# sirpkt/flink-tensorflow

Hardware: AMD Instinct MI355X
Metric: records/sec (whole node) + p50 per-record latency, ResNet-50 stream DP=1/8 (higher is better)
Workload: dtype bf16

## Files before the change

flink_tensorflow_amd/config.py:

```python
from __future__ import annotations

import argparse
import contextlib
import dataclasses
import os
from dataclasses import dataclass, field
from typing import Any

_HBM_BYTES_MI355X = 288 * 1024 ** 3


@dataclass
class EngineConfig:
    parallelism: int = 1
    max_batch: int = 256
    max_delay_ms: float = 10.0
    precision: str = "bf16"
    batch_buckets: tuple = (64, 256)
    arena_fraction: float = 0.9
    use_hip_graph: bool = True
    pipeline_depth: int = 3
    checkpoint_interval_s: float | None = None
    checkpoint_dir: str | None = None
    restart_attempts: int = 0
    restart_delay_s: float = 0.0
    channel_capacity: int = 1024
    log_level: str = "INFO"
    sibling_conv_fusion: bool = True
    fuse_preprocess_stem: bool = True
    fuse_block_tails: bool = True
    decimate_tails: bool = True
    recompute_tails: bool = True
    chain_max_links: int = 2
    pw_res_kernel: bool = True
    conv3x3c64_kernel: bool = True
    chain_batch: int = -1
    chain_min_hw: int = 5041
    chain_edge: bool = True
    wd_fused_step: bool = True
    wd_sparse_exchange: str = "owner"
    wd_bucket_slack: float = 2.0
    extra: dict = field(default_factory=dict)

    @classmethod
    def field_names(cls) -> list[str]:
        return [f.name for f in dataclasses.fields(cls) if f.name != "extra"]

    def _coerce(self, name: str, value: Any) -> Any:
        cur = getattr(self, name)
        typ = {f.name: f.type for f in dataclasses.fields(self)}[name]
        if value is None:
            return None
        if isinstance(value, str):
            if "tuple" in str(typ):
                return tuple(int(v) for v in value.replace(" ", "").split(",") if v)
            if "bool" in str(typ):
                return value.lower() in ("1", "true", "yes", "on")
            if "int" in str(typ) and "float" not in str(typ):
                return int(value)
            if "float" in str(typ):
                return float(value)
            return value
        if isinstance(cur, tuple) and isinstance(value, (list, tuple)):
            return tuple(value)
        return value

    def update(self, values: dict) -> "EngineConfig":
        for k, v in values.items():
            if k in self.field_names():
                setattr(self, k, self._coerce(k, v))
            else:
                self.extra[k] = v
        self.validate()
        return self

    @classmethod
    def from_yaml(cls, path: str, base: "EngineConfig | None" = None) -> "EngineConfig":
        import yaml

        with open(path) as f:
            data = yaml.safe_load(f) or {}
        return (base or cls()).update(data)

    @classmethod
    def from_env(cls, base: "EngineConfig | None" = None, prefix: str = "FT_", environ=None) -> "EngineConfig":
        environ = os.environ if environ is None else environ
        vals = {}
# ... 101 lines not shown
```

flink_tensorflow_amd/graph/compiler.py:

```python
from __future__ import annotations

import collections
import logging
import types
from typing import Any

import numpy as np
import torch

from ..ops import fp8 as F8
from ..ops import kernels as K
from ..types.dtypes import DataType
from ..types.names import TensorName
from ..types.tensor import StringTensor
from ..utils import tracing
from . import ops_core
from .conv_lowering import _ACTS, ConvLowering
from .graph import Graph, Node
from .op_registry import OpContext, lookup
from .ops_nn import same_pads
from .plan import CompileError, Step, Val, _buf_shape, _cfg, _coff, _eff_scale, _host, _nbytes, _root, _target, _view
from .transformer_lowering import TransformerLowering

__all__ = ["CompiledFunction", "CompileError", "Step", "Val", "compile_signature"]

LOG = logging.getLogger("flink_tensorflow_amd.compiler")

_STATS = ("fused_shortcuts", "fused_tails", "decimated_tails", "fused_pools", "conv3x3c64", "pw_res", "chained_tails",
          "conv_lite", "commuted_pools", "sibling_groups", "fused_preprocess")

_BINARY = {"Add": "add", "AddV2": "add", "Sub": "sub", "Mul": "mul", "RealDiv": "div", "Div": "div",
           "Maximum": "max", "Minimum": "min"}


class _ConstSession:

    def __init__(self, variables):
        self.variables = variables
        self._const_cache = {}


class CompiledFunction(TransformerLowering, ConvLowering):
    def __init__(self, graph: Graph, feeds: dict[str, tuple[tuple, Any]], fetches: list[str], device,
                 variables: dict | None = None, use_graph: bool = True, strict: bool = False,
                 topk_fetch: bool = True, precision: str = "bf16", calibration: dict | None = None,
                 arena=None, token_capacity: int | None = None):
        if precision not in ("bf16", "fp8"):
            raise ValueError(f"precision must be bf16 or fp8, not {precision!r}")
        from .control_flow import fold_static_control_flow
        from .functions import has_functional_ops, lower_functional_ops

        if has_functional_ops(graph):
            graph = lower_functional_ops(graph)
        graph = fold_static_control_flow(graph, list(feeds), list(fetches))
        self.graph = graph
        self.arena = arena
        self.token_cap = token_capacity
        self._pack: dict | None = None
        self._cls_nodes: set[str] = set()
        self._cur_cls = False
        self._cls_cache: dict[int, Val] = {}
        self.activation_bytes = 0
        self.precision = precision
        self.device = torch.device(device)
        if self.device.type != "cuda":
            use_graph = False
        self.feed_names = [str(TensorName.parse(f)) for f in feeds]
        self.feed_specs = {str(TensorName.parse(f)): v for f, v in feeds.items()}
        self.fetch_names = [str(TensorName.parse(f)) for f in fetches]
        self.variables = variables or {}
        self.strict = strict
        self.steps: list[Step] = []
        self.params: list[torch.Tensor] = []
        self.glue_ops: list[str] = []
        self.vals: dict[tuple[str, int], Val] = {}
        self._fused: set[str] = set()
        self._const_sess = _ConstSession(self.variables)
        self._input_bufs: dict[str, torch.Tensor] = {}
        self._outputs: list = []
        self._graph_obj: torch.cuda.CUDAGraph | None = None
        self._graph_tail: torch.cuda.CUDAGraph | None = None
        self._head: tuple[str, Step] | None = None
# ... 720 lines not shown
                    born[id(tgt)] = i
        for t in owners.values():
            t.last_use = max([t.last_use] + [c.last_use for c in getattr(t, "_concat_children", [])])
        transient = []
        for k, t in owners.items():
            if k in internal:
                continue
            if k in keep:
                t.buf = self._persistent(_buf_shape(t), t.dtype)
            else:
                transient.append(t)
        sizes = [_nbytes(_buf_shape(t), t.dtype) for t in transient]
        first = [born[id(t)] for t in transient]
        last = [max(born[id(t)], t.last_use) for t in transient]
        if chain:
            i0, i1 = chain["range"]
            for j, t in enumerate(transient):
                if id(t) in chain["touched"]:
                    if i0 <= first[j] < i1:
                        first[j] = i0
                    if last[j] >= i0:
                        last[j] = max(last[j], i1 - 1)
            chain_layout = self._plan_chain(chain, born)
            sizes.append(max(chain_layout[1], 1))
            first.append(i0)
            last.append(i1 - 1)
        offs, total = plan_offsets(sizes, first, last)
        self.activation_bytes = total
        slab = self.arena.shared_slab(total) if self.arena is not None else \
            torch.empty(max(total, 1), dtype=torch.uint8, device=self.device)
        for t, off, nb, lu in zip(transient, offs, sizes, last):
            t.buf = slab[off:off + nb].view(t.dtype).view(tuple(_buf_shape(t)))
            self._poison_after.setdefault(lu, []).append(t.buf)
        if chain:
            self._bind_chain(chain, chain_layout, slab, offs[-1])
        for v in self.vals.values():
            if v.alias_of is not None:
                r = _root(v)
                if r.buf is not None:
                    shape = v.shape if id(r) not in internal else (chain["batch"], *v.shape[1:])
                    v.buf = r.buf.view(shape) if r.buf.is_contiguous() else r.buf.reshape(shape)
        if chain:
            self._chain = (chain["range"][0], chain["range"][1], chain["parts"], chain["batch"],
                           [v for v in chain["vals"] if id(_root(v)) not in internal], chain["n"],
                           [v for v in chain["vals"] if id(_root(v)) in internal and v.buf is not None])
        self._outputs = []
        for fv in fetch_vals:
            if fv.is_const:
                self._outputs.append(fv.const)
            else:
                self._outputs.append(fv)

    _CHAIN_KINDS = ("conv", "gemm", "pool", "elementwise", "conv_fp8", "pool_fp8")
    _PERSISTENT_IMPLS = ("conv3x3c64", "bottleneck_tail", "bottleneck_chain", "pw_res")

    def _find_chain(self, keep: set) -> dict | None:
        cfg = _cfg()
        bs = int(getattr(cfg, "chain_batch", 0) or 0)
        auto = bs < 0
        if auto:
            bs = 32
        if bs == 0 or self._pack is not None or not self.steps or not self.feed_names:
            return None
        tn = TensorName.parse(self.feed_names[0])
        N = self.vals[(tn.name, tn.index)].shape[0] if self.vals[(tn.name, tn.index)].shape else 0
        if not N or -(-N // bs) < 2:
            return None
        min_hw = int(getattr(cfg, "chain_min_hw", 3136))

        edge = bool(getattr(cfg, "chain_edge", False))

        def val_ok(v):
            if v is None or v.is_const:
                return True
            r = _root(v)
            if v.rows is not None or v.concat_slot is not None or r.concat_slot is not None or r.is_const:
                return False
            if len(v.shape) != 4 or v.shape[0] != N:
                return False
            return _buf_shape(r)[0] == N

        def step_ok(st):
            vs = [v for v in list(st.inputs) + list(st.outputs) if v is not None and not v.is_const]
            if st.kind not in self._CHAIN_KINDS or not vs or not all(val_ok(v) for v in vs):
                return False
            if auto and st.meta.get("impl") in self._PERSISTENT_IMPLS:
                return False
            big = [v.shape[1] * v.shape[2] >= min_hw for v in vs]
            return any(big) if edge else all(big)

        start = 1 if self.steps[0].kind == "preprocess" else 0
        best, i = None, start
        while i < len(self.steps):
            if not step_ok(self.steps[i]):
                i += 1
                continue
            j = i
            while j < len(self.steps) and step_ok(self.steps[j]):
                j += 1
            if j - i >= 2 and (best is None or j - i > best[1] - best[0]):
                best = (i, j)
            i = j
        if best is None:
            return None
        i0, i1 = best
        vals, touched = [], set()
        for st in self.steps[i0:i1]:
# ... 280 lines not shown
```

flink_tensorflow_amd/graph/conv_lowering.py:

```python
from __future__ import annotations

from dataclasses import dataclass

import numpy as np
import torch

from ..ops import fp8 as F8
from ..ops import kernels as K
from ..types.names import TensorName
from .graph import Node
from .ops_nn import same_pads
from .plan import CompileError, Val, _cfg, _coff, _eff_scale, _root, _target, _view

_ACTS = {"Relu": K.ACT_RELU, "Relu6": K.ACT_RELU6, "Sigmoid": K.ACT_SIGMOID, "Tanh": K.ACT_TANH}

LITE_FP8_CFG = 11
_PP_MIN_K = 512

_PLAIN_ACTS = (K.ACT_NONE, K.ACT_RELU)


@dataclass(frozen=True)
class ConvSite:

# ... 302 lines not shown
                      splits=splits, ws=ws)

        self._emit(c.node.name, "gemm", run_pp, [c.xin], [c.out], {"impl": "gemm_pp"})
        self._finish_conv(c.last, c.absorbed, c.out)

    def _emit_pw_res(self, c: _ConvJob):
        w_nk = c.w_dev.reshape(c.site.cout, c.site.cin)
        bz = self._zero_bias(c)

        def run_pw(xin=c.xin, out=c.out, res_val=c.res_val, w_nk=w_nk, bz=bz):
            K.pw_res(xin.buf, w_nk, bz, res_val.buf, out=_target(out), out_channel_offset=_coff(out))

        self._emit(c.node.name, "conv", run_pw, [c.xin, c.res_val], [c.out], {"impl": "pw_res"})
        self.stats["pw_res"] += 1
        self._finish_conv(c.last, c.absorbed, c.out)

    def _emit_conv_lite(self, c: _ConvJob):
        s = c.site
        cl = K.ConvPP([(tuple(c.xin.shape), s.kernel, s.stride, (s.pads[0], s.pads[2]), s.dil)], s.cout,
                      tuple(c.out.shape[1:3]), self.device)

        def run_l(xin=c.xin, out=c.out, res_val=c.res_val, cl=cl, w2=c.w_dev.reshape(s.cout, -1), b_dev=c.b_dev):
            cl([xin.buf], w2, b_dev, res_val.buf if res_val is not None else None, s.act, out=_target(out),
               out_channel_offset=_coff(out))

        self.stats["conv_lite"] += 1
        self._emit_single_conv(c, run_l)

    def _emit_igemm(self, c: _ConvJob):
        s = c.site

        def run(xin=c.xin, out=c.out, res_val=c.res_val, w_dev=c.w_dev, b_dev=c.b_dev):
            K.conv2d_nhwc(xin.buf, w_dev, b_dev, res_val.buf if res_val is not None else None, s.stride,
                          s.pads, s.dil, s.act, out=_target(out), out_channel_offset=_coff(out),
                          out_scale=_eff_scale(out) if out.qscale is not None else None)

        self._emit_single_conv(c, run)

    def _emit_single_conv(self, c: _ConvJob, run):
        s = c.site
        shortcut_ok = (s.kernel == (1, 1) and s.stride[0] == s.stride[1] and s.pads == (0, 0, 0, 0) and s.dil == (1, 1)
                       and not s.residual and s.act == K.ACT_NONE and not s.out_fp8 and s.unpadded_cin)
        meta = {"shortcut": dict(x=c.xin, w=c.w_ohwi, bias=c.bias, stride=s.stride[0],
                                 params=[c.w_dev, c.b_dev])} if shortcut_ok else None
        self._emit(c.node.name, "conv", run, [c.xin] + ([c.res_val] if c.res_val else []), [c.out], meta)
        self._finish_conv(c.last, c.absorbed, c.out)

    def _fuse_residual_conv(self, c: _ConvJob) -> bool:
        s = c.site
        if c.res_val is None or not s.pointwise or s.s2d:
            return False
        if not s.out_fp8 and self._fuse_shortcut(c):
            return True
        return self._fuse_block_tail(c.xin, c.out, c.w_ohwi.reshape(c.w_ohwi.shape[0], -1), c.w_dev, c.b_dev,
                                     c.res_val, None, s.act, c.absorbed, c.last, c.node.name)

    def _fuse_shortcut(self, c: _ConvJob) -> bool:
        xin, out, res_val, w_ohwi, bias, act = c.xin, c.out, c.res_val, c.w_ohwi, c.bias, c.site.act
        prod = [st for st in self.steps if any(o is res_val for o in st.outputs)]
        if len(prod) != 1 or "shortcut" not in prod[0].meta or res_val.concat_slot is not None:
            return False
        for (n, _), v in self.vals.items():
            if v is res_val:
                if any(TensorName.parse(f).name == n for f in self.fetch_names):
                    return False
                if any(k != c.add_node.name and k not in self._fused for k in self.cons.get(n, [])):
                    return False
        sc = prod[0].meta["shortcut"]
        x2 = sc["x"]
        s2 = sc["stride"]
        N, Ho, Wo, _ = out.shape
        if x2.shape[0] != N or (Ho - 1) * s2 >= x2.shape[1] or (Wo - 1) * s2 >= x2.shape[2]:
            return False
        Cout, K1 = w_ohwi.shape[0], w_ohwi.shape[3]
        C2 = sc["w"].shape[3]
        if K1 % 8 or C2 % 8:
            return False
        self.steps.remove(prod[0])
        for t in sc["params"]:
            if t is not None:
                self.params = [q for q in self.params if q is not t]
        w_cat = torch.cat([w_ohwi.reshape(Cout, K1), sc["w"].reshape(Cout, C2)], 1)
        b = (bias if bias is not None else torch.zeros(Cout)) + (sc["bias"] if sc["bias"] is not None else 0)
        w_dev = self._dev(w_cat, torch.bfloat16)
        b_dev = self._dev(b, torch.float32)
        self.params += [w_dev, b_dev]
        for a in c.absorbed:
            self._fused.add(a.name)
        if not (s2 == 1 and self._fuse_block_tail(xin, out, w_cat, w_dev, b_dev, None, x2, act, c.absorbed, c.last,
                                                  c.node.name)):
            self._emit_dual(c, x2, s2, w_dev, b_dev, K1, C2)
        self.stats["fused_shortcuts"] += 1
        return True

    def _emit_dual(self, c: _ConvJob, x2: Val, s2: int, w_dev, b_dev, K1: int, C2: int):
        xin, out, act = c.xin, c.out, c.site.act
        N, Ho, Wo, Cout = out.shape
        s2cfg = {"s2": s2}
        meta = {"s2cfg": s2cfg}
        if (self.device.type == "cuda" and K1 % 64 == 0
                and C2 % 64 == 0 and (xin.phys_c or K1) == K1 and (x2.phys_c or C2) == C2
                and act in _PLAIN_ACTS and out.dtype == torch.bfloat16 and out.qscale is None
                and _coff(out) % 8 == 0 and len(xin.shape) == 4 and N * Ho * Wo <= 65536):
            xs0 = (tuple(xin.shape), (1, 1), (1, 1), (0, 0), (1, 1))
            lite = {s2: K.ConvPP([xs0, (tuple(x2.shape), (1, 1), (s2, s2), (0, 0), (1, 1))], Cout, (Ho, Wo),
                                 self.device)}
            N2, H2, W2, _ = x2.shape
            if s2 == 2 and H2 % 2 == 0 and W2 % 2 == 0:
                lite[1] = K.ConvPP([xs0, ((N2, H2 // 2, W2 // 2, C2), (1, 1), (1, 1), (0, 0), (1, 1))], Cout, (Ho, Wo),
                                   self.device)

            def run(xin=xin, x2=x2, out=out, w_dev=w_dev, b_dev=b_dev, s2cfg=s2cfg, lite=lite):
                lite[s2cfg["s2"]]([xin.buf, x2.buf], w_dev, b_dev, None, act, out=_target(out),
                                  out_channel_offset=_coff(out))

            meta["impl"] = "conv_lite_dual"
            self.stats["conv_lite"] += 1
        else:
            def run(xin=xin, x2=x2, out=out, w_dev=w_dev, b_dev=b_dev, s2cfg=s2cfg):
                K.conv1x1_dual(xin.buf, x2.buf, w_dev, b_dev, s2cfg["s2"], act, out=_target(out),
                               out_channel_offset=_coff(out))

        self._emit(c.node.name, "conv", run, [xin, x2], [out], meta)
        self._finish_conv(c.last, c.absorbed, out)

    def _fuse_block_tail(self, xin, out, w3, w_dev, b_dev, res_val, xs_val, act, absorbed, last, name) -> bool:
        if not _cfg().fuse_block_tails or self.precision == "fp8":
            return False
        cx = xin.shape[-1]
        co = 4 * cx
        widths = {64: (64, 128)}.get(cx, ()) if xs_val is None else ((64,) if cx == 64 else ())

        def plain(v):
            return v.shape[-1] == cx and (v.phys_c or cx) == cx and v.concat_slot is None and v.qscale is None \
                and v.dtype == torch.bfloat16 and tuple(v.shape[:-1]) == tuple(out.shape[:-1])

        if not widths or act != K.ACT_RELU or out.qscale is not None \
                or tuple(w3.shape) != (co, cx if xs_val is None else 2 * cx) or not plain(xin):
            return False
        if res_val is not None and (res_val.shape != out.shape or res_val.qscale is not None
                                    or res_val.concat_slot is not None):
            return False
        if xs_val is not None and not plain(xs_val):
            return False
        cand = [self.graph[c] for c in self.cons.get(last.name, []) if c not in self._fused]

        def reduce_conv(c):
            if c.op != "Conv2D" or c.inputs[0] != (last.name, 0) or c.attr("data_format", "NHWC") != "NHWC" \
                    or list(c.attr("strides")) != [1, 1, 1, 1] \
                    or list(c.attr("dilations") or [1, 1, 1, 1]) != [1, 1, 1, 1]:
                return None
            wv = self._get(c.inputs[1])
            if wv is None or not wv.is_const:
                return None
            w = wv.const.float()
            return w if tuple(w.shape[:3]) == (1, 1, co) and w.shape[3] in widths else None

        cand = [(c, w) for c in cand for w in [reduce_conv(c)] if w is not None]
        if len(cand) != 1:
            return False
        c, w2 = cand[0]
        last2, scale2, bias2, residual2, act2, absorbed2 = self._conv_chain(c)
        if residual2 is not None or act2 != K.ACT_RELU:
            return False
        cn = w2.shape[3]
        if scale2 is not None:
            w2 = w2 * scale2
        w3_dev = w_dev
        b3_dev = b_dev if b_dev is not None else self._dev(torch.zeros(co), torch.float32)
        w1_dev = self._dev(w2.reshape(co, cn).t().contiguous(), torch.bfloat16)
        b1_dev = self._dev(bias2 if bias2 is not None else torch.zeros(cn), torch.float32)
        self.params += [b3_dev, w1_dev, b1_dev]
        N, H, W, _ = out.shape
        out2 = self._new((N, H, W, cn))
        for a in absorbed + absorbed2:
            self._fused.add(a.name)
        self._fused.add(c.name)

        second = res_val if xs_val is None else xs_val
        dec = {"on": False}
        chain = {"links": None, "store": True}

        def run(xin=xin, second=second, out=out, out2=out2, dual=xs_val is not None, dec=dec, chain=chain):
            if chain["links"] is not None:
                K.bottleneck_chain([(x.buf, s.buf if s is not None else None, w, b) for x, s, w, b in chain["links"]],
                                   w1_dev, b1_dev, y1=out2.buf, y3=out.buf if chain["store"] else None,
                                   y3_decimated=dec["on"], store_y3=chain["store"])
                return
            K.bottleneck_tail(xin.buf, None if dual else second.buf, w3_dev, b3_dev, w1_dev, b1_dev, y3=out.buf,
                              y1=out2.buf, xs=second.buf if dual else None, y3_decimated=dec["on"])

        self._emit(name, "conv", run, [xin, second], [out, out2],
                   {"impl": "bottleneck_tail", "dec": dec if xs_val is None and cx == 64 else None,
                    "tail": {"x": xin, "xs": xs_val, "res": res_val, "w3": w3_dev, "b3": b3_dev, "cn": cn,
                             "chain": chain}})
        self._finish_conv(last, absorbed, out)
        self._finish_conv(last2, absorbed2, out2)
        self.stats["fused_tails"] += 1
        return True

    def _fusable_maxpool(self, last: Node, act, out: Val, fp8: bool = False):
        if act != K.ACT_RELU:
            return None
        if (out.qscale is not None or out.dtype != torch.bfloat16) if not fp8 else \
                (out.qscale is None or out.dtype != torch.uint8):
            return None
        if any(TensorName.parse(f).name == last.name for f in self.fetch_names):
            return None
        cons = [c for c in self.cons.get(last.name, []) if c not in self._fused]
        if len(cons) != 1 or self.graph[cons[0]].op != "MaxPool":
            return None
        pn = self.graph[cons[0]]
        if pn.attr("data_format", "NHWC") != "NHWC" or list(pn.attr("ksize")) != [1, 3, 3, 1] \
                or list(pn.attr("strides")) != [1, 2, 2, 1]:
            return None
        _, Ho, Wo, _ = out.shape
        if pn.attr("padding", "VALID") == "SAME":
            pt, pb = same_pads(Ho, 3, 2)
            pl, pr = same_pads(Wo, 3, 2)
        else:
            pt = pb = pl = pr = 0
        if max(pt, pb, pl, pr) > 1:
            return None
        return pn, (pt, pb, pl, pr), ((Ho + pt + pb - 3) // 2 + 1, (Wo + pl + pr - 3) // 2 + 1)

    def _conv_fp8_ok(self, node: Node, x: Val, Cin, Cout, residual, act) -> bool:
        if residual is not None or act not in _PLAIN_ACTS or Cin % 16 or Cout % 16 or x.phys_c:
            return False
        if x.qscale is not None:
            return True
        return x.dtype == torch.bfloat16 and self._qscale(node.inputs[0][0]) is not None

    def _lower_conv_fp8(self, node, x, w, bias, act, last, absorbed, kdims, stride, pads, dil, out_nhw):
        KH, KW, Cin, Cout = kdims
        w_ohwi = w.permute(3, 0, 1, 2).contiguous()
        wq, ws = F8.quantize_weight(w_ohwi)
        x_scale = x.qscale if x.qscale is not None else self._qscale(node.inputs[0][0])
        wq_dev = self._dev(wq)
        ws_dev = self._dev(ws)
        cs_dev = self._dev(ws * x_scale, torch.float32)
        b_dev = self._dev(bias, torch.float32) if bias is not None else \
            torch.zeros(Cout, dtype=torch.float32, device=self.device)
        self.params += [wq_dev, cs_dev, b_dev]
        o_scale = self._qscale(last.name) if self._fp8_consumers_ok(last.name) else None
        out = self._new((*out_nhw, Cout), torch.uint8 if o_scale is not None else torch.bfloat16)
        out.qscale = o_scale
        for a in absorbed:
            self._fused.add(a.name)
        self.fp8_layers += 1
        site = ConvSite(on_gpu=self.device.type == "cuda", x_shape=tuple(x.shape), cin=Cin, cin_phys=Cin, cout=Cout,
                        kernel=(KH, KW), stride=tuple(stride), pads=tuple(pads), dil=tuple(dil), act=act,
# ... 245 lines not shown
            F8.avgpool_bias_act(y.buf, ksize, (1, 1), pads, b, act,
                                out_scale=_eff_scale(out) if out.qscale is not None else None, out=_target(out),
                                out_channel_offset=_coff(out))

        self._emit(node.name, "pool_fp8" if o_scale is not None else "pool", run_pool, [y], [out],
                   {"impl": "avgpool_bias_act"})
        self._fused.add(c.name)
        for a in absorbed:
            self._fused.add(a.name)
        self._finish_conv(last, absorbed, out)
        self.stats["commuted_pools"] += 1
        return True

    def _fetched_roots(self) -> set:
        return {id(_root(self.vals[(TensorName.parse(f).name, TensorName.parse(f).index)])) for f in self.fetch_names}

    def _chain_tails(self):
        if not _cfg().recompute_tails:
            return
        fetched = self._fetched_roots()
        links_of: dict[int, list] = {}
        for st in self.steps:
            t = st.meta.get("tail")
            if t is None or t["w3"] is None:
                continue
            if t["xs"] is not None:
                links_of[id(st)] = [(t["x"], t["xs"], t["w3"], t["b3"])]
                continue
            res = t["res"]
            prods = [p for p in self.steps if p.outputs and p.outputs[0] is res and id(p) in links_of]
            if len(prods) != 1:
                continue
            prev = prods[0]
            prev_links = links_of[id(prev)]
            if len(prev_links) >= _cfg().chain_max_links or id(res) in fetched or res.alias_of is not None or res.concat_slot is not None \
                    or res.buf_shape is not None \
                    or any(v is not res and _root(v) is res for v in self.vals.values()):
                continue
            readers = [r for r in self.steps if r is not prev and any(_root(i) is res for i in r.inputs)]
            if readers != [st]:
                continue
            links = prev_links + [(t["x"], None, t["w3"], t["b3"])]
            links_of[id(st)] = links
            t["chain"]["links"] = links
            st.meta["impl"] = "bottleneck_chain"
            st.inputs = [v for x, xs, _, _ in links for v in ((x,) if xs is None else (x, xs))]
            pt = prev.meta["tail"]
            pt["chain"]["links"] = prev_links
            pt["chain"]["store"] = False
            prev.meta["impl"] = "bottleneck_chain"
            prev.outputs = [o for o in prev.outputs if o is not res]
            self.stats["chained_tails"] += 1

    def _decimate_tails(self):
        if not _cfg().decimate_tails:
            return
        fetched = self._fetched_roots()
        for st in self.steps:
            dec = st.meta.get("dec")
            if dec is None:
                continue
            y3 = st.outputs[0]
            if id(y3) in fetched or y3.alias_of is not None or y3.concat_slot is not None \
                    or y3.buf_shape is not None:
                continue
            if any(v is not y3 and _root(v) is y3 for v in self.vals.values()):
                continue
            readers = [r for r in self.steps if r is not st and any(_root(i) is y3 for i in r.inputs)]
            if len(readers) != 1:
                continue
            r = readers[0]
            cfg = (r.meta or {}).get("s2cfg")
            N, H, W, C = y3.shape
            if cfg is None or cfg["s2"] != 2 or len(r.inputs) != 2 or r.inputs[1] is not y3 or H % 2 or W % 2 \
                    or tuple(r.outputs[0].shape[1:3]) != (H // 2, W // 2):
                continue
            y3.buf_shape = (N, H // 2, W // 2, C)
            dec["on"] = True
            cfg["s2"] = 1
            self.stats["decimated_tails"] += 1
```

flink_tensorflow_amd/kernels/module.hip:

```cpp
#include <pybind11/pybind11.h>
#include <hip/hip_runtime.h>

#include <cstdint>
#include <stdexcept>
#include <string>

void register_igemm(pybind11::module_& m);
void register_nn_misc(pybind11::module_& m);
void register_transformer(pybind11::module_& m);
void register_embedding(pybind11::module_& m);
void register_fp8(pybind11::module_& m);
void register_attention(pybind11::module_& m);
void register_dconv(pybind11::module_& m);
void register_elementwise(pybind11::module_& m);
void register_conv3x3c64(pybind11::module_& m);
void register_bottleneck(pybind11::module_& m);
void register_bottleneck_chain(pybind11::module_& m);
void register_gemm_pp(pybind11::module_& m);
void register_conv_pp(pybind11::module_& m);
void register_widedeep(pybind11::module_& m);
void register_sort_segments(pybind11::module_& m);
void register_pw_res(pybind11::module_& m);
void register_gemm_train(pybind11::module_& m);

PYBIND11_MODULE(_hip, m) {
  m.doc() = "flink_tensorflow_amd CDNA4 (gfx950) kernels";
  m.attr("arch") = "gfx950";
  register_igemm(m);
  register_nn_misc(m);
  register_transformer(m);
  register_embedding(m);
  register_fp8(m);
  register_attention(m);
  register_dconv(m);
  register_elementwise(m);
  register_conv3x3c64(m);
  register_bottleneck(m);
  register_bottleneck_chain(m);
  register_gemm_pp(m);
  register_conv_pp(m);
  register_widedeep(m);
  register_sort_segments(m);
  register_pw_res(m);
  register_gemm_train(m);
  m.def("stream_create", [](int priority) {
    hipStream_t s = nullptr;
    hipError_t e = hipStreamCreateWithPriority(&s, hipStreamNonBlocking, priority);
    if (e != hipSuccess) throw std::runtime_error(std::string("hipStreamCreateWithPriority: ") + hipGetErrorString(e));
    return reinterpret_cast<std::uintptr_t>(s);
  }, pybind11::arg("priority") = 0);
  m.def("stream_destroy", [](std::uintptr_t s) {
    hipError_t e = hipStreamDestroy(reinterpret_cast<hipStream_t>(s));
    if (e != hipSuccess) throw std::runtime_error(std::string("hipStreamDestroy: ") + hipGetErrorString(e));
  });
}
```

flink_tensorflow_amd/ops/kernels.py:

```python
from __future__ import annotations

import copy
import functools
import os

import torch
import torch.nn.functional as F

from .. import _ext

ACT_NONE, ACT_RELU, ACT_GELU, ACT_SIGMOID, ACT_TANH, ACT_RELU6, ACT_DRELU = 0, 1, 2, 3, 4, 5, 6
_ACT_NAMES = {None: ACT_NONE, "none": ACT_NONE, "relu": ACT_RELU, "gelu": ACT_GELU, "gelu_tanh": ACT_GELU,
              "sigmoid": ACT_SIGMOID, "tanh": ACT_TANH, "relu6": ACT_RELU6, "drelu": ACT_DRELU}


def act_code(act) -> int:
    if isinstance(act, int):
        return act
    try:
        return _ACT_NAMES[act]
    except KeyError:
        raise ValueError(f"unknown activation {act!r}") from None


# ... 156 lines not shown
        return out
    return conv2d_nhwc(x, w_ohwi, bias, None, (1, 1), (1, 1, 1, 1), (1, 1), a, out=out,
                       out_channel_offset=out_channel_offset)


def bottleneck_tail(x2: torch.Tensor, res: torch.Tensor | None, w3: torch.Tensor, b3: torch.Tensor, w1: torch.Tensor,
                    b1: torch.Tensor, y3: torch.Tensor | None = None, y1: torch.Tensor | None = None,
                    xs: torch.Tensor | None = None, y3_decimated: bool = False):
    lead = x2.shape[:-1]
    dec_hw = (0, 0)
    if y3_decimated:
        if x2.dim() != 4 or x2.shape[1] % 2 or x2.shape[2] % 2 or x2.shape[-1] != 64:
            raise ValueError("bottleneck_tail: decimated y3 needs x2 [N, H, W, 64] with even H, W")
        dec_hw = (x2.shape[1], x2.shape[2])
    dual = xs is not None
    cx = x2.shape[-1]
    co = 4 * cx
    cn = w1.shape[0]
    if (res is None) != dual:
        raise ValueError("bottleneck_tail: pass exactly one of res and xs")
    if (cx, dual, cn) not in ((64, True, 64), (64, False, 64), (64, False, 128)):
        raise ValueError(f"bottleneck_tail: unsupported variant x2 [..., {cx}], dual {dual}, reduce width {cn}")
    k3 = 2 * cx if dual else cx
    if (dual and tuple(xs.shape) != (*lead, cx)) or (not dual and tuple(res.shape) != (*lead, co)):
        raise ValueError(f"bottleneck_tail: the second input must be [..., {cx if dual else co}]")
    if tuple(w3.reshape(w3.shape[0], -1).shape) != (co, k3) or tuple(w1.reshape(cn, -1).shape) != (cn, co):
        raise ValueError(f"bottleneck_tail: weights must be [{co}, {k3}] and [{cn}, {co}], got {tuple(w3.shape)} "
                         f"{tuple(w1.shape)}")
    if b3.numel() != co or b1.numel() != cn:
        raise ValueError("bottleneck_tail: bias sizes must match the output channels")
    odt = x2.dtype if x2.is_cuda else torch.float32
    lead3 = (lead[0], dec_hw[0] // 2, dec_hw[1] // 2) if y3_decimated else lead
    y3 = torch.empty((*lead3, co), dtype=odt, device=x2.device) if y3 is None else y3
    y1 = torch.empty((*lead, cn), dtype=odt, device=x2.device) if y1 is None else y1
    if tuple(y3.shape) != (*lead3, co) or tuple(y1.shape) != (*lead, cn):
        raise ValueError("bottleneck_tail: output buffers do not fit")
    M = x2.numel() // cx
    second = xs if dual else res
    if x2.is_cuda:
        for t, n in ((x2, "x2"), (second, "xs" if dual else "res"), (w3, "w3"), (w1, "w1"), (y3, "y3"), (y1, "y1")):
            _check(t, n, device=x2.device)
        _check(b3, "b3", torch.float32, x2.device)
        _check(b1, "b1", torch.float32, x2.device)
        dev = x2.device.index if x2.device.index is not None else torch.cuda.current_device()
        _hip().bottleneck_tail_bf16(x2.data_ptr(), _ptr(xs), _ptr(res), w3.data_ptr(), b3.data_ptr(),
                                    w1.data_ptr(), b1.data_ptr(), y3.data_ptr(), y1.data_ptr(), M, cn,
                                    _NUM_CU[dev], _stream(), dec_hw[0], dec_hw[1])
        return y3, y1
    xin = torch.cat([x2.reshape(M, cx), xs.reshape(M, cx)], 1) if dual else x2.reshape(M, cx)
    a = xin.float() @ w3.reshape(co, k3).float().t() + b3.float()
    a = a.to(odt).float()
    a = torch.relu(a if dual else a + res.reshape(M, co).float()).to(y3.dtype)
    y3.copy_(a.reshape(*lead, co)[:, ::2, ::2] if y3_decimated else a.reshape(y3.shape))
    b = torch.relu(a.float() @ w1.reshape(cn, co).float().t() + b1.float())
    y1.copy_(b.reshape(y1.shape).to(y1.dtype))
    return y3, y1


def bottleneck_chain(links, w1: torch.Tensor, b1: torch.Tensor, y1: torch.Tensor | None = None,
                     y3: torch.Tensor | None = None, y3_decimated: bool = False, store_y3: bool = True):
    x0 = links[0][0]
    lead = x0.shape[:-1]
    M = x0.numel() // 64
    cn = w1.shape[0]
    if not 1 <= len(links) <= 3 or links[0][1] is None or any(l[1] is not None for l in links[1:]):
        raise ValueError("bottleneck_chain: 1 to 3 links, the first dual ([x | xs]), the others plain")
    for j, (x, xs, w, b) in enumerate(links):
        if x.shape[-1] != 64 or x.numel() != M * 64 or (xs is not None and tuple(xs.shape) != tuple(x.shape)):
            raise ValueError("bottleneck_chain: every source is [..., 64] over the same pixels")
        if tuple(w.reshape(w.shape[0], -1).shape) != (256, 128 if j == 0 else 64) or b.numel() != 256:
            raise ValueError(f"bottleneck_chain: link {j} weights must be [256, {128 if j == 0 else 64}]")
    if cn not in (64, 128) or tuple(w1.reshape(cn, -1).shape) != (cn, 256) or b1.numel() != cn:
        raise ValueError("bottleneck_chain: w1 must be [64 or 128, 256]")
    dec_hw = (0, 0)
    if y3_decimated:
        if x0.dim() != 4 or x0.shape[1] % 2 or x0.shape[2] % 2:
            raise ValueError("bottleneck_chain: decimated y3 needs [N, H, W, 64] sources with even H, W")
        dec_hw = (x0.shape[1], x0.shape[2])
    odt = x0.dtype if x0.is_cuda else torch.float32
    lead3 = (lead[0], dec_hw[0] // 2, dec_hw[1] // 2) if y3_decimated else lead
    if store_y3 and y3 is None:
        y3 = torch.empty((*lead3, 256), dtype=odt, device=x0.device)
    y1 = torch.empty((*lead, cn), dtype=odt, device=x0.device) if y1 is None else y1
    if (store_y3 and tuple(y3.shape) != (*lead3, 256)) or tuple(y1.shape) != (*lead, cn):
        raise ValueError("bottleneck_chain: output buffers do not fit")
    if x0.is_cuda:
        for j, (x, xs, w, b) in enumerate(links):
            for t, n in ((x, "x"), (w, "w")) + (((xs, "xs"),) if xs is not None else ()):
                _check(t, f"link {j} {n}", device=x0.device)
            _check(b, f"link {j} bias", torch.float32, x0.device)
        _check(w1, "w1", device=x0.device)
        _check(b1, "b1", torch.float32, x0.device)
        _check(y1, "y1", device=x0.device)
        if store_y3:
            _check(y3, "y3", device=x0.device)
        dev = x0.device.index if x0.device.index is not None else torch.cuda.current_device()
        _hip().bottleneck_chain_bf16([(x.data_ptr(), _ptr(xs), w.data_ptr(), b.data_ptr()) for x, xs, w, b in links],
                                     w1.data_ptr(), b1.data_ptr(), y3.data_ptr() if store_y3 else 0, y1.data_ptr(), M,
                                     cn, _NUM_CU[dev], _stream(), dec_hw[0], dec_hw[1])
        return (y3 if store_y3 else None), y1
    y = None
    rdt = y1.dtype
    for x, xs, w, b in links:
        xin = torch.cat([x.reshape(M, 64), xs.reshape(M, 64)], 1) if xs is not None else x.reshape(M, 64)
        a = (xin.float() @ w.reshape(256, -1).float().t() + b.float()).to(odt).float()
        y = torch.relu(a if y is None else a + y).to(rdt).float()
# ... 802 lines not shown
```

Before: 82620.

## Fuse ResNet stage-2 block tail with next block's 1x1 reduce conv

Adds a persistent HIP kernel that fuses the 128->512 expand conv, bias, residual add and ReLU with the following 512->128 reduce conv for ResNet stage-2 blocks. The intermediate 512-channel activation stays in LDS for the second GEMM instead of being re-read from HBM, and weights are streamed in slices via buffer-load-to-LDS. It is gated by a minimum row count, by default 128 rows times the CU count. This adds a large hand-scheduled kernel with counted waitcnt assumptions that could be fragile.

```diff
diff --git a/flink_tensorflow_amd/config.py b/flink_tensorflow_amd/config.py
--- a/flink_tensorflow_amd/config.py
+++ b/flink_tensorflow_amd/config.py
@@ -33,6 +33,8 @@
     recompute_tails: bool = True
     chain_max_links: int = 2
     pw_res_kernel: bool = True
+    fuse_wide_tails: bool = True
+    wide_tail_min_rows: int = -1
     conv3x3c64_kernel: bool = True
     chain_batch: int = -1
     chain_min_hw: int = 5041
diff --git a/flink_tensorflow_amd/graph/compiler.py b/flink_tensorflow_amd/graph/compiler.py
--- a/flink_tensorflow_amd/graph/compiler.py
+++ b/flink_tensorflow_amd/graph/compiler.py
@@ -27,7 +27,7 @@
 LOG = logging.getLogger("flink_tensorflow_amd.compiler")
 
 _STATS = ("fused_shortcuts", "fused_tails", "decimated_tails", "fused_pools", "conv3x3c64", "pw_res", "chained_tails",
-          "conv_lite", "commuted_pools", "sibling_groups", "fused_preprocess")
+          "wide_tails", "conv_lite", "commuted_pools", "sibling_groups", "fused_preprocess")
 
 _BINARY = {"Add": "add", "AddV2": "add", "Sub": "sub", "Mul": "mul", "RealDiv": "div", "Div": "div",
            "Maximum": "max", "Minimum": "min"}
@@ -854,7 +854,7 @@
                 self._outputs.append(fv)
 
     _CHAIN_KINDS = ("conv", "gemm", "pool", "elementwise", "conv_fp8", "pool_fp8")
-    _PERSISTENT_IMPLS = ("conv3x3c64", "bottleneck_tail", "bottleneck_chain", "pw_res")
+    _PERSISTENT_IMPLS = ("conv3x3c64", "bottleneck_tail", "bottleneck_chain", "pw_res", "wide_tail")
 
     def _find_chain(self, keep: set) -> dict | None:
         cfg = _cfg()
diff --git a/flink_tensorflow_amd/graph/conv_lowering.py b/flink_tensorflow_amd/graph/conv_lowering.py
--- a/flink_tensorflow_amd/graph/conv_lowering.py
+++ b/flink_tensorflow_amd/graph/conv_lowering.py
@@ -378,8 +378,12 @@
             return False
         if not s.out_fp8 and self._fuse_shortcut(c):
             return True
-        return self._fuse_block_tail(c.xin, c.out, c.w_ohwi.reshape(c.w_ohwi.shape[0], -1), c.w_dev, c.b_dev,
-                                     c.res_val, None, s.act, c.absorbed, c.last, c.node.name)
+        w3 = c.w_ohwi.reshape(c.w_ohwi.shape[0], -1)
+        if self._fuse_block_tail(c.xin, c.out, w3, c.w_dev, c.b_dev, c.res_val, None, s.act, c.absorbed, c.last,
+                                 c.node.name):
+            return True
+        return not s.out_fp8 and self._fuse_wide_tail(c.xin, c.out, w3, c.w_dev, c.b_dev, c.res_val, s.act,
+                                                      c.absorbed, c.last, c.node.name)
 
     def _fuse_shortcut(self, c: _ConvJob) -> bool:
         xin, out, res_val, w_ohwi, bias, act = c.xin, c.out, c.res_val, c.w_ohwi, c.bias, c.site.act
@@ -469,6 +473,45 @@
             return False
         if xs_val is not None and not plain(xs_val):
             return False
+        red = self._tail_reduce(last, co, widths)
+        if red is None:
+            return False
+        c, w2, bias2, last2, absorbed2 = red
+        cn = w2.shape[3]
+        w3_dev = w_dev
+        b3_dev = b_dev if b_dev is not None else self._dev(torch.zeros(co), torch.float32)
+        w1_dev = self._dev(w2.reshape(co, cn).t().contiguous(), torch.bfloat16)
+        b1_dev = self._dev(bias2 if bias2 is not None else torch.zeros(cn), torch.float32)
+        self.params += [b3_dev, w1_dev, b1_dev]
+        N, H, W, _ = out.shape
+        out2 = self._new((N, H, W, cn))
+        for a in absorbed + absorbed2:
+            self._fused.add(a.name)
+        self._fused.add(c.name)
+
+        second = res_val if xs_val is None else xs_val
+        dec = {"on": False}
+        chain = {"links": None, "store": True}
+
+        def run(xin=xin, second=second, out=out, out2=out2, dual=xs_val is not None, dec=dec, chain=chain):
+            if chain["links"] is not None:
+                K.bottleneck_chain([(x.buf, s.buf if s is not None else None, w, b) for x, s, w, b in chain["links"]],
+                                   w1_dev, b1_dev, y1=out2.buf, y3=out.buf if chain["store"] else None,
+                                   y3_decimated=dec["on"], store_y3=chain["store"])
+                return
+            K.bottleneck_tail(xin.buf, None if dual else second.buf, w3_dev, b3_dev, w1_dev, b1_dev, y3=out.buf,
+                              y1=out2.buf, xs=second.buf if dual else None, y3_decimated=dec["on"])
+
+        self._emit(name, "conv", run, [xin, second], [out, out2],
+                   {"impl": "bottleneck_tail", "dec": dec if xs_val is None and cx == 64 else None,
+                    "tail": {"x": xin, "xs": xs_val, "res": res_val, "w3": w3_dev, "b3": b3_dev, "cn": cn,
+                             "chain": chain}})
+        self._finish_conv(last, absorbed, out)
+        self._finish_conv(last2, absorbed2, out2)
+        self.stats["fused_tails"] += 1
+        return True
+
+    def _tail_reduce(self, last: Node, co: int, widths):
         cand = [self.graph[c] for c in self.cons.get(last.name, []) if c not in self._fused]
 
         def reduce_conv(c):
@@ -484,15 +527,36 @@
 
         cand = [(c, w) for c in cand for w in [reduce_conv(c)] if w is not None]
         if len(cand) != 1:
-            return False
+            return None
         c, w2 = cand[0]
         last2, scale2, bias2, residual2, act2, absorbed2 = self._conv_chain(c)
         if residual2 is not None or act2 != K.ACT_RELU:
-            return False
-        cn = w2.shape[3]
+            return None
         if scale2 is not None:
             w2 = w2 * scale2
-        w3_dev = w_dev
+        return c, w2, bias2, last2, absorbed2
+
+    def _fuse_wide_tail(self, xin, out, w3, w_dev, b_dev, res_val, act, absorbed, last, name) -> bool:
+        cfg = _cfg()
+        if not cfg.fuse_wide_tails or self.precision == "fp8":
+            return False
+        cx, co, cn = 128, 512, 128
+
+        def plain(v, ch):
+            return v.shape[-1] == ch and (v.phys_c or ch) == ch and v.concat_slot is None and v.qscale is None \
+                and v.dtype == torch.bfloat16 and tuple(v.shape[:-1]) == tuple(out.shape[:-1])
+
+        if act != K.ACT_RELU or out.qscale is not None or out.concat_slot is not None or out.dtype != torch.bfloat16 \
+                or tuple(w3.shape) != (co, cx) or not plain(xin, cx) or res_val is None or not plain(res_val, co) \
+                or tuple(out.shape) != tuple(res_val.shape):
+            return False
+        if int(np.prod(out.shape[:-1])) < self._wide_tail_min_rows():
+            return False
+        red = self._tail_reduce(last, co, (cn,))
+        if red is None:
+            return False
+        c, w2, bias2, last2, absorbed2 = red
+        w3_dev = w_dev.reshape(co, cx)
         b3_dev = b_dev if b_dev is not None else self._dev(torch.zeros(co), torch.float32)
         w1_dev = self._dev(w2.reshape(co, cn).t().contiguous(), torch.bfloat16)
         b1_dev = self._dev(bias2 if bias2 is not None else torch.zeros(cn), torch.float32)
@@ -503,26 +567,13 @@
             self._fused.add(a.name)
         self._fused.add(c.name)
 
-        second = res_val if xs_val is None else xs_val
-        dec = {"on": False}
-        chain = {"links": None, "store": True}
-
-        def run(xin=xin, second=second, out=out, out2=out2, dual=xs_val is not None, dec=dec, chain=chain):
-            if chain["links"] is not None:
-                K.bottleneck_chain([(x.buf, s.buf if s is not None else None, w, b) for x, s, w, b in chain["links"]],
-                                   w1_dev, b1_dev, y1=out2.buf, y3=out.buf if chain["store"] else None,
-                                   y3_decimated=dec["on"], store_y3=chain["store"])
-                return
-            K.bottleneck_tail(xin.buf, None if dual else second.buf, w3_dev, b3_dev, w1_dev, b1_dev, y3=out.buf,
-                              y1=out2.buf, xs=second.buf if dual else None, y3_decimated=dec["on"])
-
-        self._emit(name, "conv", run, [xin, second], [out, out2],
-                   {"impl": "bottleneck_tail", "dec": dec if xs_val is None and cx == 64 else None,
-                    "tail": {"x": xin, "xs": xs_val, "res": res_val, "w3": w3_dev, "b3": b3_dev, "cn": cn,
-                             "chain": chain}})
+        def run(xin=xin, res_val=res_val, out=out, out2=out2):
+            K.wide_tail(xin.buf, res_val.buf, w3_dev, b3_dev, w1_dev, b1_dev, y3=out.buf, y1=out2.buf)
+
+        self._emit(name, "conv", run, [xin, res_val], [out, out2], {"impl": "wide_tail"})
         self._finish_conv(last, absorbed, out)
         self._finish_conv(last2, absorbed2, out2)
-        self.stats["fused_tails"] += 1
+        self.stats["wide_tails"] += 1
         return True
 
     def _fusable_maxpool(self, last: Node, act, out: Val, fp8: bool = False):
@@ -874,6 +925,15 @@
             prev.outputs = [o for o in prev.outputs if o is not res]
             self.stats["chained_tails"] += 1
 
+    def _wide_tail_min_rows(self) -> int:
+        n = _cfg().wide_tail_min_rows
+        if n >= 0:
+            return n
+        dev = self.device
+        ncu = K._NUM_CU[dev.index if dev.index is not None else torch.cuda.current_device()] \
+            if dev.type == "cuda" else 256
+        return K.WIDE_TAIL_TP * ncu
+
     def _decimate_tails(self):
         if not _cfg().decimate_tails:
             return
diff --git a/flink_tensorflow_amd/kernels/module.hip b/flink_tensorflow_amd/kernels/module.hip
--- a/flink_tensorflow_amd/kernels/module.hip
+++ b/flink_tensorflow_amd/kernels/module.hip
@@ -21,6 +21,7 @@
 void register_widedeep(pybind11::module_& m);
 void register_sort_segments(pybind11::module_& m);
 void register_pw_res(pybind11::module_& m);
+void register_wide_tail(pybind11::module_& m);
 void register_gemm_train(pybind11::module_& m);
 
 PYBIND11_MODULE(_hip, m) {
@@ -42,6 +43,7 @@
   register_widedeep(m);
   register_sort_segments(m);
   register_pw_res(m);
+  register_wide_tail(m);
   register_gemm_train(m);
   m.def("stream_create", [](int priority) {
     hipStream_t s = nullptr;
diff --git a/flink_tensorflow_amd/kernels/wide_tail.hip b/flink_tensorflow_amd/kernels/wide_tail.hip
--- /dev/null
+++ b/flink_tensorflow_amd/kernels/wide_tail.hip
@@ -0,0 +1,238 @@
+#include <pybind11/pybind11.h>
+
+#include <stdexcept>
+#include <string>
+
+#include "common.h"
+
+namespace {
+
+constexpr int NT = 512;
+constexpr int CX = 128;
+constexpr int CO = 512;
+constexpr int CN = 128;
+constexpr int TP = 128;
+constexpr int BS = 128;
+constexpr int NS = CO / BS;
+constexpr int CPR = 16;
+constexpr int TILE_BYTES = 128 * 128 * 2;
+constexpr int IT = TP * CPR / NT;
+
+FTM_DEVICE int swz(int row, int c) { return row * CPR + (c ^ (row & 15)); }
+
+#define WT_FENCE() asm volatile("" ::: "memory")
+#define WT_BARRIER()                              \
+  do {                                            \
+    __builtin_amdgcn_sched_barrier(0);            \
+    asm volatile("s_barrier" ::: "memory");       \
+    __builtin_amdgcn_sched_barrier(0);            \
+  } while (0)
+#define WT_SYNC_LDS()                                      \
+  do {                                                     \
+    asm volatile("s_waitcnt lgkmcnt(0)" ::: "memory");     \
+    WT_BARRIER();                                          \
+  } while (0)
+
+__global__ __launch_bounds__(NT, 1) void wide_tail_kernel(const bf16* x, const bf16* res, const bf16* __restrict__ w3,
+                                                          const float* __restrict__ b3, const bf16* __restrict__ w1,
+                                                          const float* __restrict__ b1, bf16* y3, bf16* y1, int M) {
+  extern __shared__ __attribute__((aligned(1024))) uint8_t smem[];
+  u32x4* Xs = reinterpret_cast<u32x4*>(smem);
+  u32x4* Ys = reinterpret_cast<u32x4*>(smem + TILE_BYTES);
+  uint8_t* W3b = smem + 2 * TILE_BYTES;
+  uint8_t* W1b = smem + 3 * TILE_BYTES;
+  const u32x4* W3s = reinterpret_cast<const u32x4*>(W3b);
+  const u32x4* W1s = reinterpret_cast<const u32x4*>(W1b);
+  float* Bs = reinterpret_cast<float*>(smem + 4 * TILE_BYTES);
+  const int tid = threadIdx.x, lane = tid & 63;
+  const int wave = __builtin_amdgcn_readfirstlane(tid >> 6);
+  const int prow = lane & 15, kg = lane >> 4;
+  const int wp = wave >> 2, wc = wave & 3;
+  const int tiles = (M + TP - 1) / TP;
+  int t = blockIdx.x;
+  if (t >= tiles) return;
+
+  unsigned off3[4], off1[4];
+#pragma unroll
+  for (int k0 = 0; k0 < 4; ++k0) {
+    const int row = (wave * 4 + k0) * 4 + (lane >> 4);
+    const int c = (lane & 15) ^ (row & 15);
+    off3[k0] = (unsigned)(row * CX + c * 8) * 2u;
+    off1[k0] = (unsigned)(row * CO + c * 8) * 2u;
+  }
+  const __amdgpu_buffer_rsrc_t rs3 = __builtin_amdgcn_make_buffer_rsrc((void*)w3, 0, CO * CX * 2, 0x00020000);
+  const __amdgpu_buffer_rsrc_t rs1 = __builtin_amdgcn_make_buffer_rsrc((void*)w1, 0, CN * CO * 2, 0x00020000);
+  auto dma_w = [&](__amdgpu_buffer_rsrc_t rs, int slice_bytes, const unsigned (&off)[4], uint8_t* dst) {
+#pragma unroll
+    for (int k0 = 0; k0 < 4; ++k0)
+      __builtin_amdgcn_raw_ptr_buffer_load_lds(rs, (__attribute__((address_space(3))) void*)(dst + (wave * 4 + k0) * 1024),
+                                               16, off[k0], slice_bytes, 0, 0);
+  };
+  const int crow = tid >> 4, cch = tid & 15;
+  u32x4 xr[IT], rv[2][IT];
+  auto load_x = [&](int tt) {
+#pragma unroll
+    for (int it = 0; it < IT; ++it) {
+      const int px = min(tt * TP + crow + it * 32, M - 1);
+      xr[it] = reinterpret_cast<const u32x4*>(x + (size_t)px * CX)[cch];
+    }
+  };
+  auto store_x = [&]() {
+#pragma unroll
+    for (int it = 0; it < IT; ++it) Xs[swz(crow + it * 32, cch)] = xr[it];
+  };
+  auto load_r = [&](u32x4 (&r)[IT], int tt, int s) {
+#pragma unroll
+    for (int it = 0; it < IT; ++it) {
+      const int px = min(tt * TP + crow + it * 32, M - 1);
+      r[it] = reinterpret_cast<const u32x4*>(res + (size_t)px * CO + s * BS)[cch];
+    }
+  };
+
+  dma_w(rs3, 0, off3, W3b);
+  load_x(t);
+  load_r(rv[0], t, 0);
+  store_x();
+  for (int q = tid; q < CO + CN; q += NT) Bs[q] = q < CO ? b3[q] : b1[q - CO];
+  asm volatile("s_waitcnt vmcnt(0) lgkmcnt(0)" ::: "memory");
+  __syncthreads();
+
+  while (true) {
+    const int p0 = t * TP;
+    const int tn = t + (int)gridDim.x;
+    f32x4 acc2[2][4];
+#pragma unroll
+    for (int i = 0; i < 2; ++i)
+#pragma unroll
+      for (int j = 0; j < 4; ++j) acc2[i][j] = f32x4{0.f, 0.f, 0.f, 0.f};
+#pragma unroll
+    for (int s = 0; s < NS; ++s) {
+      dma_w(rs1, s * BS * 2, off1, W1b);
+      WT_FENCE();
+      load_r(rv[(s + 1) & 1], s == NS - 1 ? tn : t, (s + 1) % NS);
+      if (s == 1) load_x(tn);
+      WT_FENCE();
+      f32x4 acc[2][4];
+#pragma unroll
+      for (int i = 0; i < 2; ++i)
+#pragma unroll
+        for (int j = 0; j < 4; ++j) acc[i][j] = f32x4{0.f, 0.f, 0.f, 0.f};
+#pragma unroll
+      for (int ks = 0; ks < CX / 32; ++ks) {
+        if (ks == 2) __builtin_amdgcn_sched_barrier(0);
+        const int c = ks * 4 + kg;
+        bf16x8 a[2], bb[4];
+#pragma unroll
+        for (int i = 0; i < 2; ++i) a[i] = __builtin_bit_cast(bf16x8, W3s[swz(wc * 32 + i * 16 + prow, c)]);
+#pragma unroll
+        for (int j = 0; j < 4; ++j) bb[j] = __builtin_bit_cast(bf16x8, Xs[swz(wp * 64 + j * 16 + prow, c)]);
+#pragma unroll
+        for (int i = 0; i < 2; ++i)
+#pragma unroll
+          for (int j = 0; j < 4; ++j) acc[i][j] = __builtin_amdgcn_mfma_f32_16x16x32_bf16(a[i], bb[j], acc[i][j], 0, 0, 0);
+      }
+#pragma unroll
+      for (int i = 0; i < 2; ++i) {
+        const int co = wc * 32 + i * 16 + kg * 4;
+        const f32x4 bv = *reinterpret_cast<const f32x4*>(Bs + s * BS + co);
+#pragma unroll
+        for (int j = 0; j < 4; ++j) {
+          bf16x4 o;
+#pragma unroll
+          for (int r = 0; r < 4; ++r) o[r] = f2bf(acc[i][j][r] + bv[r]);
+          bf16* chunk = reinterpret_cast<bf16*>(Ys + swz(wp * 64 + j * 16 + prow, co >> 3));
+          *reinterpret_cast<bf16x4*>(chunk + (co & 7)) = o;
+        }
+      }
+      if (s == 1) asm volatile("s_waitcnt vmcnt(8) lgkmcnt(0)" ::: "memory");
+      else asm volatile("s_waitcnt vmcnt(4) lgkmcnt(0)" ::: "memory");
+      static_assert(IT == 4, "the counted waits above assume 4 prefetch loads per tile per thread");
+      WT_BARRIER();
+#pragma unroll
+      for (int it = 0; it < IT; ++it) {
+        const int pl = crow + it * 32;
+        const int si = swz(pl, cch);
+        bf16x8 v = __builtin_bit_cast(bf16x8, Ys[si]);
+        const bf16x8 r = __builtin_bit_cast(bf16x8, rv[s & 1][it]);
+#pragma unroll
+        for (int e = 0; e < 8; ++e) v[e] = f2bf(fmaxf((float)v[e] + (float)r[e], 0.f));
+        Ys[si] = __builtin_bit_cast(u32x4, v);
+        if (p0 + pl < M)
+          *reinterpret_cast<u32x4*>(y3 + (size_t)(p0 + pl) * CO + s * BS + cch * 8) = __builtin_bit_cast(u32x4, v);
+      }
+      WT_FENCE();
+      dma_w(rs3, ((s + 1) % NS) * BS * CX * 2, off3, W3b);
+      if (s == NS - 1) store_x();
+      WT_SYNC_LDS();
+#pragma unroll
+      for (int ks = 0; ks < BS / 32; ++ks) {
+        if (ks == 2) __builtin_amdgcn_sched_barrier(0);
+        const int c = ks * 4 + kg;
+        bf16x8 a[2], bb[4];
+#pragma unroll
+        for (int i = 0; i < 2; ++i) a[i] = __builtin_bit_cast(bf16x8, W1s[swz(wc * 32 + i * 16 + prow, c)]);
+#pragma unroll
+        for (int j = 0; j < 4; ++j) bb[j] = __builtin_bit_cast(bf16x8, Ys[swz(wp * 64 + j * 16 + prow, c)]);
+#pragma unroll
+        for (int i = 0; i < 2; ++i)
+#pragma unroll
+          for (int j = 0; j < 4; ++j)
+            acc2[i][j] = __builtin_amdgcn_mfma_f32_16x16x32_bf16(a[i], bb[j], acc2[i][j], 0, 0, 0);
+      }
+      asm volatile("s_waitcnt vmcnt(0) lgkmcnt(0)" ::: "memory");
+      WT_BARRIER();
+    }
+#pragma unroll
+    for (int i = 0; i < 2; ++i) {
+      const int co = wc * 32 + i * 16 + kg * 4;
+      const f32x4 bv = *reinterpret_cast<const f32x4*>(Bs + CO + co);
+#pragma unroll
+      for (int j = 0; j < 4; ++j) {
+        bf16x4 o;
+#pragma unroll
+        for (int r = 0; r < 4; ++r) o[r] = f2bf(fmaxf(acc2[i][j][r] + bv[r], 0.f));
+        bf16* chunk = reinterpret_cast<bf16*>(Ys + swz(wp * 64 + j * 16 + prow, co >> 3));
+        *reinterpret_cast<bf16x4*>(chunk + (co & 7)) = o;
+      }
+    }
+    WT_SYNC_LDS();
+#pragma unroll
+    for (int it = 0; it < IT; ++it) {
+      const int pl = crow + it * 32;
+      if (p0 + pl < M) reinterpret_cast<u32x4*>(y1 + (size_t)(p0 + pl) * CN)[cch] = Ys[swz(pl, cch)];
+    }
+    if (tn >= tiles) break;
+    WT_SYNC_LDS();
+    t = tn;
+  }
+}
+
+}
+
+static void wide_tail_check(std::initializer_list<uintptr_t> ptrs, int M, int grid, int tp) {
+  if (M <= 0) throw std::invalid_argument("wide_tail: empty problem");
+  if (grid <= 0) throw std::invalid_argument("wide_tail: grid must be positive");
+  if ((long)M * CO >= (1L << 31)) throw std::invalid_argument("wide_tail: tensor too large for 32-bit indexing");
+  for (uintptr_t p : ptrs)
+    if (!p || p % 16) throw std::invalid_argument("wide_tail: null or non-16-byte-aligned pointer");
+  if (((long)((M + tp - 1) / tp) + (long)grid) * tp >= (1L << 31)) throw std::invalid_argument("wide_tail: grid too large");
+}
+
+void wide_tail_bf16(uintptr_t x, uintptr_t res, uintptr_t w3, uintptr_t b3, uintptr_t w1, uintptr_t b1, uintptr_t y3,
+                    uintptr_t y1, int M, int grid, uintptr_t stream) {
+  wide_tail_check({x, res, w3, b3, w1, b1, y3, y1}, M, grid, TP);
+  const int tiles = (M + TP - 1) / TP;
+  const int g = grid < tiles ? grid : tiles;
+  constexpr size_t lds = 4 * TILE_BYTES + (CO + CN) * 4;
+  static_assert(lds <= 160 * 1024, "LDS");
+  (void)hipFuncSetAttribute((const void*)wide_tail_kernel, hipFuncAttributeMaxDynamicSharedMemorySize, lds);
+  auto bp = [](uintptr_t p) { return reinterpret_cast<bf16*>(p); };
+  auto fp = [](uintptr_t p) { return reinterpret_cast<const float*>(p); };
+  hipLaunchKernelGGL(wide_tail_kernel, dim3(g), dim3(NT), lds, reinterpret_cast<hipStream_t>(stream), bp(x), bp(res),
+                     bp(w3), fp(b3), bp(w1), fp(b1), bp(y3), bp(y1), M);
+  FTM_CHECK_LAUNCH();
+}
+
+void register_wide_tail(pybind11::module_& m) {
+  m.def("wide_tail_bf16", &wide_tail_bf16);
+}
diff --git a/flink_tensorflow_amd/ops/kernels.py b/flink_tensorflow_amd/ops/kernels.py
--- a/flink_tensorflow_amd/ops/kernels.py
+++ b/flink_tensorflow_amd/ops/kernels.py
@@ -232,6 +232,49 @@
     a = a.to(odt).float()
     a = torch.relu(a if dual else a + res.reshape(M, co).float()).to(y3.dtype)
     y3.copy_(a.reshape(*lead, co)[:, ::2, ::2] if y3_decimated else a.reshape(y3.shape))
+    b = torch.relu(a.float() @ w1.reshape(cn, co).float().t() + b1.float())
+    y1.copy_(b.reshape(y1.shape).to(y1.dtype))
+    return y3, y1
+
+
+WIDE_TAIL_TP = 128
+
+
+def wide_tail(x: torch.Tensor, res: torch.Tensor, w3: torch.Tensor, b3: torch.Tensor, w1: torch.Tensor,
+              b1: torch.Tensor, y3: torch.Tensor | None = None, y1: torch.Tensor | None = None,
+              grid: int | None = None):
+    cx, co, cn = 128, 512, 128
+    lead = tuple(x.shape[:-1])
+    if x.shape[-1] != cx or tuple(res.shape) != (*lead, co):
+        raise ValueError(f"wide_tail: x must be [..., {cx}] and res [..., {co}], got {tuple(x.shape)} "
+                         f"{tuple(res.shape)}")
+    if tuple(w3.reshape(w3.shape[0], -1).shape) != (co, cx) or tuple(w1.reshape(w1.shape[0], -1).shape) != (cn, co):
+        raise ValueError(f"wide_tail: weights must be [{co}, {cx}] and [{cn}, {co}], got {tuple(w3.shape)} "
+                         f"{tuple(w1.shape)}")
+    if b3.numel() != co or b1.numel() != cn:
+        raise ValueError("wide_tail: bias sizes must match the output channels")
+    if grid is not None and not 1 <= grid <= 1 << 20:
+        raise ValueError("wide_tail: grid must be in [1, 2^20]")
+    odt = x.dtype if x.is_cuda else torch.float32
+    y3 = torch.empty((*lead, co), dtype=odt, device=x.device) if y3 is None else y3
+    y1 = torch.empty((*lead, cn), dtype=odt, device=x.device) if y1 is None else y1
+    if tuple(y3.shape) != (*lead, co) or tuple(y1.shape) != (*lead, cn):
+        raise ValueError("wide_tail: output buffers do not fit")
+    M = x.numel() // cx
+    if x.is_cuda:
+        for t, n in ((x, "x"), (res, "res"), (w3, "w3"), (w1, "w1"), (y3, "y3"), (y1, "y1")):
+            _check(t, n, device=x.device)
+        _check(b3, "b3", torch.float32, x.device)
+        _check(b1, "b1", torch.float32, x.device)
+        dev = x.device.index if x.device.index is not None else torch.cuda.current_device()
+        _hip().wide_tail_bf16(x.data_ptr(), res.data_ptr(), w3.data_ptr(), b3.data_ptr(), w1.data_ptr(),
+                              b1.data_ptr(), y3.data_ptr(), y1.data_ptr(), M, _NUM_CU[dev] if grid is None else grid,
+                              _stream())
+        return y3, y1
+    a = x.reshape(M, cx).float() @ w3.reshape(co, cx).float().t() + b3.float()
+    a = a.to(odt).float()
+    a = torch.relu(a + res.reshape(M, co).float()).to(y3.dtype)
+    y3.copy_(a.reshape(y3.shape))
     b = torch.relu(a.float() @ w1.reshape(cn, co).float().t() + b1.float())
     y1.copy_(b.reshape(y1.shape).to(y1.dtype))
     return y3, y1
```

After: 83420 (median of 6 runs). No clear change (+1.0%).
